# NIFTy-PPL/NIFTy

Measured on AMD Instinct MI355X. Metric: MGVI iters/sec on 1024^3 RGSpace CorrelatedField, 8 samples; achieved HBM GB/s, higher is better.
Workload: dtype f32

## Files before the change

__graft_entry__.py:

```python
import os
import subprocess
import sys

ROOT = os.path.dirname(os.path.abspath(__file__))
if ROOT not in sys.path:
    sys.path.insert(0, ROOT)


def build():
    csrc = os.path.join(ROOT, "nifty_amd", "csrc")
    subprocess.check_call(["make", "-C", csrc, "-j4", "ARCH=gfx950"])
    subprocess.check_call(["make", "-C", csrc, "fence", "ARCH=gfx950"])
    emu_dir = os.path.join(ROOT, "tests", "emu")
    subprocess.check_call(["g++", "-O2", "-std=c++17", "-shared", "-fPIC", "-o",
                           os.path.join(emu_dir, "libnk_emu.so"), os.path.join(emu_dir, "emu_fft.cpp"),
                           os.path.join(emu_dir, "emu_rng.cpp")])
    import oracle.nifty_oracle

    import nifty_amd
    from nifty_amd import _lib

    lib = _lib.load()
    assert lib.nk_version() >= 100


def smoke():
    import numpy as np
    import torch

    from nifty_amd import random
    from nifty_amd.engine import FusedKL, FusedModel, LatentVec, draw_samples
    from nifty_amd.minimization import AbsDeltaEnergyController
    from oracle import nifty_oracle as orc

    assert torch.cuda.is_available(), "smoke() needs a GPU"
    shape = (64, 64, 128)
    rng = np.random.default_rng(0)
    cf = orc.CFModel(shape, None, orc.CFParams(offset_mean=2.0))
    x = {k: 0.2 * v for k, v in cf.draw_latent(rng).items()}
    v = cf.draw_latent(rng)
    data = cf.forward(cf.draw_latent(rng)) + 0.1 * rng.normal(size=shape)
    lh = orc.Likelihood("gaussian", data, icov=100.0)
    lin = orc.Linearized(cf, lh, x)
    val, grad = lin.value_grad()
    mv = lin.metric(v)

    model = FusedModel(shape, offset_mean=2.0, likelihood="gaussian", data=data, icov=100.0, device="cuda:0")
    xl, vl = LatentVec.from_dict(model, x), LatentVec.from_dict(model, v)
    lp = model.linearize(xl)

    def rel(a, b):
        return max(float(np.max(np.abs(a[k] - b[k])) / max(np.max(np.abs(b[k])), 1e-30)) for k in ("xi", "spectrum"))

    assert abs(float(lp.value.item()) - val) < 1e-10 * abs(val)
    assert rel(lp.grad.to_dict(), grad) < 1e-9
    assert model.sandwich, "the sandwich pipeline should serve this grid"
    assert rel(model.metric(lp, vl).to_dict(), mv) < 1e-9
    random.push_sseq_from_seed(7)
    res, negs, n_total = draw_samples(model, xl, 1, True, lambda: AbsDeltaEnergyController(0.05, iteration_limit=5))
    random.pop_sseq()
    res_o, negs_o = orc.draw_samples(cf, lh, x, 1, True, np.random.SeedSequence(7),
                                     lambda: orc.AbsDeltaEnergyController(0.05, iteration_limit=5))
    assert rel(res[0].to_dict(), res_o[0]) < 1e-7
    kl = FusedKL(model, xl, res, negs)
    kl_o = orc.SampledKL(cf, lh, x, res_o, negs_o)
    assert abs(kl.value - kl_o.value) < 1e-8 * abs(kl_o.value)
    print("smoke OK: value", float(lp.value.item()), "KL", kl.value)


if __name__ == "__main__":
    build()
    print("build OK")
```

nifty_amd/csrc/nk_rng.h:

```cpp
#pragma once
#include <math.h>
#include <stdint.h>

#include "nk_core.h"
#include "nk_ziggurat_tables.h"

#define NK_RNG_CHUNK 64
#define NK_RNG_ERR_NOMERGE 1u
#define NK_RNG_ERR_SHORT 2u
#define NK_ZIG_R 3.6541528853610087963519472518
#define NK_ZIG_INV_R 0.27366123732975827203338247596

struct NkU128 {
  uint64_t hi, lo;
};
NK_HD uint64_t nk_mulhi64(uint64_t a, uint64_t b) {
#if defined(__HIP_DEVICE_COMPILE__)
  return __umul64hi(a, b);
#else
  return (uint64_t)(((unsigned __int128)a * b) >> 64);
#endif
}
NK_HD NkU128 nk_mul128(NkU128 a, NkU128 b) {
  NkU128 r;
  r.lo = a.lo * b.lo;
  r.hi = nk_mulhi64(a.lo, b.lo) + a.hi * b.lo + a.lo * b.hi;
  return r;
}
NK_HD NkU128 nk_add128(NkU128 a, NkU128 b) {
  NkU128 r;
  r.lo = a.lo + b.lo;
  r.hi = a.hi + b.hi + (r.lo < a.lo ? 1u : 0u);
  return r;
}

struct NkPcgJump {
  NkU128 m[64], p[64];
};
NK_HD void nk_pcg_jump_table(NkU128 inc, NkPcgJump& t) {
  NkU128 m{0x2360ED051FC65DA4ull, 0x4385DF649FCCF645ull}, p = inc;
  for (int i = 0; i < 64; ++i) {
    t.m[i] = m;
    t.p[i] = p;
    p = nk_mul128(nk_add128(m, NkU128{0, 1}), p);
    m = nk_mul128(m, m);
  }
}
NK_HD NkU128 nk_pcg_advance(NkU128 s, uint64_t delta, const NkPcgJump& t) {
  NkU128 am{0, 1}, ap{0, 0};
  for (int i = 0; delta; ++i, delta >>= 1)
    if (delta & 1) {
      am = nk_mul128(am, t.m[i]);
      ap = nk_add128(nk_mul128(ap, t.m[i]), t.p[i]);
    }
  return nk_add128(nk_mul128(am, s), ap);
}

struct NkRaw {
  NkU128 s, inc;
  int pos;
  NK_HD uint64_t next() {
    s = nk_add128(nk_mul128(s, NkU128{0x2360ED051FC65DA4ull, 0x4385DF649FCCF645ull}), inc);
    ++pos;
    const uint64_t x = s.hi ^ s.lo;
    const unsigned rot = (unsigned)(s.hi >> 58);
    return (x >> rot) | (x << ((64u - rot) & 63u));
  }
  NK_HD double next_double() { return (double)(next() >> 11) * (1.0 / 9007199254740992.0); }
};

struct NkZig {
  const uint64_t* ki;
  const double *wi, *fi;
};

#if defined(__clang__)
#define NK_NO_CONTRACT _Pragma("clang fp contract(off)")
#else
#define NK_NO_CONTRACT
#endif
#define NK_DMUL(a, b) ((a) * (b))
#define NK_DADD(a, b) ((a) + (b))

NK_HD double nk_zig_normal(NkRaw& g, const NkZig& z) {
  NK_NO_CONTRACT
  for (;;) {
    uint64_t r = g.next();
    const int idx = (int)(r & 0xff);
    r >>= 8;
    const int sign = (int)(r & 1);
    const uint64_t rabs = (r >> 1) & 0x000fffffffffffffull;
    double x = NK_DMUL((double)rabs, z.wi[idx]);
    if (sign) x = -x;
    if (rabs < z.ki[idx]) return x;
    if (idx == 0) {
      for (;;) {
        const double xx = NK_DMUL(-NK_ZIG_INV_R, log1p(-g.next_double()));
        const double yy = -log1p(-g.next_double());
        if (NK_DADD(yy, yy) > NK_DMUL(xx, xx)) return ((rabs >> 8) & 1) ? -NK_DADD(NK_ZIG_R, xx) : NK_DADD(NK_ZIG_R, xx);
      }
    } else {
      const double lhs = NK_DADD(NK_DMUL(z.fi[idx - 1] - z.fi[idx], g.next_double()), z.fi[idx]);
      if (lhs < exp(NK_DMUL(NK_DMUL(-0.5, x), x))) return x;
    }
  }
}

struct NkRngArgs {
  NkU128 state, inc;
  int64_t n;
  int64_t nchunks;
  double mean, std;
};

NK_HD NkRaw nk_rng_chunk_start(const NkRngArgs& a, const NkPcgJump& jt, int64_t k, int entry) {
  NkRaw g;
  g.inc = a.inc;
  g.s = nk_pcg_advance(a.state, (uint64_t)k * NK_RNG_CHUNK + (uint64_t)entry, jt);
  g.pos = entry;
  return g;
}

NK_HD void nk_rng_pass_a(const NkRngArgs& a, const NkPcgJump& jt, const NkZig& z, int64_t k, int& c0, int& ov, uint64_t& m) {
  NkRaw g = nk_rng_chunk_start(a, jt, k, 0);
  m = 0;
  c0 = 0;
  while (g.pos < NK_RNG_CHUNK) {
    m |= 1ull << g.pos;
    (void)nk_zig_normal(g, z);
    ++c0;
  }
  ov = g.pos - NK_RNG_CHUNK;
  if (ov > 255) ov = 255;
}

NK_HD int nk_rng_pass_a2(const NkRngArgs& a, const NkPcgJump& jt, const NkZig& z, int64_t k, int e, int c0, uint64_t m,
                         unsigned* err) {
  if (e == 0) return c0;
  if (e >= NK_RNG_CHUNK) {
    *err |= NK_RNG_ERR_NOMERGE;
    return 0;
  }
  NkRaw g = nk_rng_chunk_start(a, jt, k, e);
  int c = 0;
  while (g.pos < NK_RNG_CHUNK && !((m >> g.pos) & 1)) {
    (void)nk_zig_normal(g, z);
    ++c;
  }
  if (g.pos >= NK_RNG_CHUNK) {
    *err |= NK_RNG_ERR_NOMERGE;
    return 0;
  }
  int before = 0;
  for (int b = 0; b < g.pos; ++b) before += (int)((m >> b) & 1);
  return c + c0 - before;
}

template <typename T>
NK_HD void nk_rng_pass_b(const NkRngArgs& a, const NkPcgJump& jt, const NkZig& z, int64_t k, int entry, int64_t off, T* out,
                         uint64_t* consumed) {
  NK_NO_CONTRACT
  if (off >= a.n || entry >= NK_RNG_CHUNK) return;
  NkRaw g = nk_rng_chunk_start(a, jt, k, entry);
  while (g.pos < NK_RNG_CHUNK && off < a.n) {
    const double x = nk_zig_normal(g, z);
    out[off] = (T)NK_DADD(a.mean, NK_DMUL(a.std, x));
    if (off == a.n - 1) *consumed = (uint64_t)k * NK_RNG_CHUNK + (uint64_t)g.pos;
    ++off;
  }
}

static inline int64_t nk_rng_chunks_for(int64_t n, int attempt) {
  const double need = (double)n * (1.0225 + 0.005 * (double)(1 << attempt)) / NK_RNG_CHUNK;
  return (int64_t)need + 32 * (int64_t)(1 + attempt);
}

#define NK_RNG_FIX 32
template <typename T, int MODE>
NK_HD void nk_rng_fixed_body(NkU128 state, NkU128 inc, const NkPcgJump& jt, int64_t n, double low, double scale, int64_t k,
                             T* out) {
  NK_NO_CONTRACT
  const int64_t per = MODE == 0 ? NK_RNG_FIX : 2 * NK_RNG_FIX;
  const int64_t e0 = k * per;
  if (e0 >= n) return;
  NkRaw g;
  g.s = nk_pcg_advance(state, (uint64_t)k * NK_RNG_FIX, jt);
  g.inc = inc;
  g.pos = 0;
  for (int i = 0; i < NK_RNG_FIX; ++i) {
    const uint64_t raw = g.next();
    if (MODE == 0) {
      const int64_t e = e0 + i;
      if (e >= n) return;
      const double u = (double)(raw >> 11) * (1.0 / 9007199254740992.0);
      out[e] = (T)NK_DADD(low, NK_DMUL(scale, u));
    } else {
      for (int h = 0; h < 2; ++h) {
        const int64_t e = e0 + 2 * i + h;
        if (e >= n) return;
        const uint32_t half = h ? (uint32_t)(raw >> 32) : (uint32_t)raw;
        if (MODE == 1) {
          out[e] = (half >> 31) ? (T)1 : (T)-1;
        } else {
          const uint32_t code = half >> 30;
          out[2 * e] = code == 0 ? (T)1 : code == 2 ? (T)-1 : (T)0;
          out[2 * e + 1] = code == 1 ? (T)1 : code == 3 ? (T)-1 : (T)0;
        }
      }
    }
  }
}

struct NkIntArgs {
  NkU128 state, inc;
  int64_t n;
  uint64_t rng;
  int64_t low;
  int wide;
  uint64_t threshold;
};
NK_HD bool nk_int_accept(const NkIntArgs& a, uint64_t word, int64_t& value) {
  if (!a.wide) {
    const uint32_t excl = (uint32_t)a.rng + 1u;
    if (excl == 0u) {
      value = a.low + (int64_t)word;
      return true;
    }
    const uint64_t m = word * (uint64_t)excl;
    value = a.low + (int64_t)(m >> 32);
    return (uint32_t)m >= (uint32_t)a.threshold;
  }
  const uint64_t excl = a.rng + 1ull;
  if (excl == 0ull) {
    value = (int64_t)((uint64_t)a.low + word);
    return true;
  }
  const uint64_t lo = word * excl, hi = nk_mulhi64(word, excl);
  value = (int64_t)((uint64_t)a.low + hi);
  return lo >= a.threshold;
}
template <typename F>
NK_HD void nk_int_thread_words(const NkIntArgs& a, const NkPcgJump& jt, int64_t k, F f) {
  NkRaw g;
  g.s = nk_pcg_advance(a.state, (uint64_t)k * NK_RNG_FIX, jt);
  g.inc = a.inc;
  g.pos = 0;
  const int per = a.wide ? NK_RNG_FIX : 2 * NK_RNG_FIX;
  uint64_t raw = 0;
  for (int i = 0; i < per; ++i) {
    uint64_t word;
    if (a.wide) {
      word = g.next();
    } else {
      if ((i & 1) == 0) raw = g.next();
      word = (i & 1) ? (raw >> 32) : (raw & 0xffffffffull);
    }
    int64_t v;
    const bool ok = nk_int_accept(a, word, v);
    if (!f(k * per + i, ok, v)) return;
  }
}
NK_HD int nk_int_count(const NkIntArgs& a, const NkPcgJump& jt, int64_t k) {
  int c = 0;
  nk_int_thread_words(a, jt, k, [&](int64_t, bool ok, int64_t) {
    c += ok ? 1 : 0;
    return true;
  });
  return c;
}
NK_HD void nk_int_write(const NkIntArgs& a, const NkPcgJump& jt, int64_t k, int64_t off, int64_t* out, uint64_t* words_used) {
  nk_int_thread_words(a, jt, k, [&](int64_t word_index, bool ok, int64_t v) {
    if (!ok) return true;
    if (off >= a.n) return false;
    out[off] = v;
    if (off == a.n - 1) *words_used = (uint64_t)word_index + 1;
    ++off;
    return true;
  });
}
```

nifty_amd/csrc/nk_rng.hip:

```cpp
#include <hip/hip_runtime.h>

#include "nk_rng.h"
#include "nk_util.h"

namespace {

constexpr int RNG_THREADS = 256;

__device__ const uint64_t NK_ZIG_KI_DEV[256] = NK_ZIG_KI_INIT;
__device__ const uint64_t NK_ZIG_WI_DEV[256] = NK_ZIG_WI_BITS_INIT;
__device__ const uint64_t NK_ZIG_FI_DEV[256] = NK_ZIG_FI_BITS_INIT;

struct RngLds {
  NkPcgJump jt;
  uint64_t ki[256];
  double wi[256], fi[256];
};

__global__ void k_rng_table(NkU128 inc, NkPcgJump* out) {
  nk_pcg_jump_table(inc, *out);
}

__device__ __forceinline__ NkZig rng_load_lds(RngLds& l, const NkPcgJump* jt) {
  const uint64_t* src = (const uint64_t*)jt;
  uint64_t* dst = (uint64_t*)&l.jt;
  for (int i = threadIdx.x; i < (int)(sizeof(NkPcgJump) / 8); i += blockDim.x) dst[i] = src[i];
  for (int i = threadIdx.x; i < 256; i += blockDim.x) {
    l.ki[i] = NK_ZIG_KI_DEV[i];
    l.wi[i] = __longlong_as_double((long long)NK_ZIG_WI_DEV[i]);
    l.fi[i] = __longlong_as_double((long long)NK_ZIG_FI_DEV[i]);
  }
  __syncthreads();
  return NkZig{l.ki, l.wi, l.fi};
}

__global__ void __launch_bounds__(RNG_THREADS) k_rng_count(NkRngArgs a, const NkPcgJump* jt, uint8_t* over, uint8_t* cnt,
                                                           uint32_t* bsum, uint64_t* status) {
  __shared__ RngLds l;
  __shared__ int s_over[RNG_THREADS];
  __shared__ int s_sum[RNG_THREADS / 64];
  const NkZig z = rng_load_lds(l, jt);
  const int64_t k = (int64_t)blockIdx.x * RNG_THREADS + threadIdx.x;
  int c0 = 0, ov = 0;
  uint64_t m = 0;
  if (k < a.nchunks) nk_rng_pass_a(a, l.jt, z, k, c0, ov, m);
  s_over[threadIdx.x] = ov;
  __syncthreads();
  int c = 0;
  if (k < a.nchunks) {
    int e = 0;
    if (threadIdx.x > 0) {
      e = s_over[threadIdx.x - 1];
    } else if (k > 0) {
      int pc;
      uint64_t pm;
      nk_rng_pass_a(a, l.jt, z, k - 1, pc, e, pm);
    }
    unsigned err = 0;
    c = nk_rng_pass_a2(a, l.jt, z, k, e, c0, m, &err);
    if (err) atomicOr((unsigned long long*)&status[1], (unsigned long long)err);
    over[k] = (uint8_t)ov;
    cnt[k] = (uint8_t)c;
  }
  for (int d = 32; d > 0; d >>= 1) c += __shfl_down(c, d);
  if ((threadIdx.x & 63) == 0) s_sum[threadIdx.x >> 6] = c;
  __syncthreads();
  if (threadIdx.x == 0) {
    int t = 0;
    for (int w = 0; w < RNG_THREADS / 64; ++w) t += s_sum[w];
    bsum[blockIdx.x] = (uint32_t)t;
  }
}

__global__ void __launch_bounds__(1024) k_rng_scan(const uint32_t* bsum, int64_t nblk, int64_t n, int64_t* boff, uint64_t* status) {
  __shared__ int64_t part[1024];
  const int64_t seg = (nblk + 1023) / 1024;
  const int64_t lo = (int64_t)threadIdx.x * seg, hi = lo + seg < nblk ? lo + seg : nblk;
  int64_t s = 0;
  for (int64_t i = lo; i < hi; ++i) s += bsum[i];
  part[threadIdx.x] = s;
  __syncthreads();
  for (int d = 1; d < 1024; d <<= 1) {
    const int64_t v = threadIdx.x >= d ? part[threadIdx.x - d] : 0;
    __syncthreads();
    part[threadIdx.x] += v;
    __syncthreads();
  }
  int64_t run = part[threadIdx.x] - s;
  for (int64_t i = lo; i < hi; ++i) {
    boff[i] = run;
    run += bsum[i];
  }
  if (threadIdx.x == 1023 && part[1023] < n) atomicOr((unsigned long long*)&status[1], (unsigned long long)NK_RNG_ERR_SHORT);
}

template <typename T>
__global__ void __launch_bounds__(RNG_THREADS) k_rng_write(NkRngArgs a, const NkPcgJump* jt, const uint8_t* over, const uint8_t* cnt,
                                                           const int64_t* boff, T* out, uint64_t* status) {
  __shared__ RngLds l;
  __shared__ int s_scan[RNG_THREADS];
  const NkZig z = rng_load_lds(l, jt);
  const int64_t k = (int64_t)blockIdx.x * RNG_THREADS + threadIdx.x;
  const int c = k < a.nchunks ? cnt[k] : 0;
  s_scan[threadIdx.x] = c;
  __syncthreads();
  for (int d = 1; d < RNG_THREADS; d <<= 1) {
    const int v = threadIdx.x >= d ? s_scan[threadIdx.x - d] : 0;
    __syncthreads();
    s_scan[threadIdx.x] += v;
    __syncthreads();
  }
  if (k >= a.nchunks) return;
  const int64_t off = boff[blockIdx.x] + s_scan[threadIdx.x] - c;
  const int entry = k > 0 ? over[k - 1] : 0;
  nk_rng_pass_b<T>(a, l.jt, z, k, entry, off, out, &status[0]);
}

__global__ void __launch_bounds__(RNG_THREADS) k_int_count(NkIntArgs a, const NkPcgJump* jt, int64_t nthreads, uint8_t* cnt, uint32_t* bsum) {
  __shared__ NkPcgJump l_jt;
  __shared__ int s_sum[RNG_THREADS / 64];
  for (int i = threadIdx.x; i < (int)(sizeof(NkPcgJump) / sizeof(uint64_t)); i += blockDim.x)
    reinterpret_cast<uint64_t*>(&l_jt)[i] = reinterpret_cast<const uint64_t*>(jt)[i];
  __syncthreads();
  const int64_t k = (int64_t)blockIdx.x * RNG_THREADS + threadIdx.x;
  int c = 0;
  if (k < nthreads) {
    c = nk_int_count(a, l_jt, k);
    cnt[k] = (uint8_t)c;
  }
  for (int d = 32; d > 0; d >>= 1) c += __shfl_down(c, d);
  if ((threadIdx.x & 63) == 0) s_sum[threadIdx.x >> 6] = c;
  __syncthreads();
  if (threadIdx.x == 0) {
    int t = 0;
    for (int w = 0; w < RNG_THREADS / 64; ++w) t += s_sum[w];
    bsum[blockIdx.x] = (uint32_t)t;
  }
}
__global__ void __launch_bounds__(RNG_THREADS) k_int_write(NkIntArgs a, const NkPcgJump* jt, int64_t nthreads, const uint8_t* cnt,
                                                           const int64_t* boff, int64_t* out, uint64_t* status) {
  __shared__ NkPcgJump l_jt;
  __shared__ int s_scan[RNG_THREADS];
  for (int i = threadIdx.x; i < (int)(sizeof(NkPcgJump) / sizeof(uint64_t)); i += blockDim.x)
    reinterpret_cast<uint64_t*>(&l_jt)[i] = reinterpret_cast<const uint64_t*>(jt)[i];
  const int64_t k = (int64_t)blockIdx.x * RNG_THREADS + threadIdx.x;
  const int c = k < nthreads ? cnt[k] : 0;
  s_scan[threadIdx.x] = c;
  __syncthreads();
  for (int d = 1; d < RNG_THREADS; d <<= 1) {
    const int v = threadIdx.x >= d ? s_scan[threadIdx.x - d] : 0;
    __syncthreads();
    s_scan[threadIdx.x] += v;
    __syncthreads();
  }
  if (k >= nthreads) return;
  const int64_t off = boff[blockIdx.x] + s_scan[threadIdx.x] - c;
  if (off < a.n) nk_int_write(a, l_jt, k, off, out, &status[0]);
}

struct RngLayout {
  int64_t nchunks, nblk;
  int64_t o_over, o_cnt, o_bsum, o_boff, o_table, total;
};
RngLayout rng_layout(int64_t n, int attempt) {
  RngLayout L;
  L.nchunks = nk_rng_chunks_for(n, attempt);
  L.nblk = (L.nchunks + RNG_THREADS - 1) / RNG_THREADS;
  auto up = [](int64_t v) { return (v + 255) / 256 * 256; };
  L.o_over = 0;
  L.o_cnt = up(L.o_over + L.nchunks);
  L.o_bsum = up(L.o_cnt + L.nchunks);
  L.o_boff = up(L.o_bsum + 4 * L.nblk);
  L.o_table = up(L.o_boff + 8 * L.nblk);
  L.total = up(L.o_table + (int64_t)sizeof(NkPcgJump));
  return L;
}

template <typename T, int MODE>
__global__ void __launch_bounds__(256) k_rng_fixed(NkU128 state, NkU128 inc, const NkPcgJump* jt, int64_t n, double low,
                                                   double scale, T* out) {
  __shared__ NkPcgJump l_jt;
  for (int i = threadIdx.x; i < (int)(sizeof(NkPcgJump) / sizeof(uint64_t)); i += blockDim.x)
    reinterpret_cast<uint64_t*>(&l_jt)[i] = reinterpret_cast<const uint64_t*>(jt)[i];
  __syncthreads();
  nk_rng_fixed_body<T, MODE>(state, inc, l_jt, n, low, scale, (int64_t)blockIdx.x * blockDim.x + threadIdx.x, out);
}

template <int MODE>
int rng_fixed_launch(const uint64_t* state, const uint64_t* inc, int64_t n, double low, double scale, void* out, int dtype,
                     void* scratch, hipStream_t stream, const char* what) {
  if (!state || !inc || n < 0 || (n > 0 && (!out || !scratch)) || (dtype != NK_F32 && dtype != NK_F64))
    return nk_set_error(NK_ERR_INVALID, "nk_pcg64 fixed-rate draw: bad argument");
  if (!(inc[1] & 1)) return nk_set_error(NK_ERR_INVALID, "nk_pcg64 fixed-rate draw: the increment of a PCG64 stream is odd");
  if (n == 0) return NK_OK;
  const NkU128 s{state[0], state[1]}, c{inc[0], inc[1]};
  NkPcgJump* jt = (NkPcgJump*)scratch;
  hipLaunchKernelGGL(k_rng_table, dim3(1), dim3(1), 0, stream, c, jt);
  const int64_t per = MODE == 0 ? NK_RNG_FIX : 2 * NK_RNG_FIX;
  const int64_t threads = (n + per - 1) / per;
  const unsigned blocks = (unsigned)((threads + 255) / 256);
  if (dtype == NK_F32)
    hipLaunchKernelGGL((k_rng_fixed<float, MODE>), dim3(blocks), dim3(256), 0, stream, s, c, jt, n, low, scale, (float*)out);
  else
    hipLaunchKernelGGL((k_rng_fixed<double, MODE>), dim3(blocks), dim3(256), 0, stream, s, c, jt, n, low, scale, (double*)out);
  return nk_check_launch(what);
}

}

extern "C" int64_t nk_pcg64_fixed_scratch_bytes(void) { return (int64_t)sizeof(NkPcgJump); }

extern "C" int nk_pcg64_uniform(const uint64_t* state, const uint64_t* inc, int64_t n, double low, double high, void* out,
                                int dtype, void* scratch, void* stream) {
  return rng_fixed_launch<0>(state, inc, n, low, high - low, out, dtype, scratch, (hipStream_t)stream, "nk_pcg64_uniform");
}

extern "C" int nk_pcg64_pm1(const uint64_t* state, const uint64_t* inc, int64_t n, void* out, int dtype, int complex_units,
                            void* scratch, void* stream) {
  if (complex_units)
    return rng_fixed_launch<2>(state, inc, n, 0.0, 0.0, out, dtype, scratch, (hipStream_t)stream, "nk_pcg64_pm1");
  return rng_fixed_launch<1>(state, inc, n, 0.0, 0.0, out, dtype, scratch, (hipStream_t)stream, "nk_pcg64_pm1");
}

extern "C" int64_t nk_pcg64_integers_scratch_bytes(int64_t nthreads) {
  if (nthreads < 0) return 0;
  auto up = [](int64_t v) { return (v + 255) / 256 * 256; };
  const int64_t nblk = (nthreads + RNG_THREADS - 1) / RNG_THREADS;
  return up(nthreads) + up(4 * nblk) + up(8 * nblk) + up((int64_t)sizeof(NkPcgJump));
}

extern "C" int nk_pcg64_integers(const uint64_t* state, const uint64_t* inc, int64_t n, int64_t low, uint64_t rng, int64_t nthreads,
                                 int64_t* out, void* scratch, uint64_t* status, void* stream_) {
  hipStream_t stream = (hipStream_t)stream_;
  if (!state || !inc || n < 0 || nthreads < 0 || !status || (n > 0 && (!out || !scratch || nthreads < 1)) || rng == 0)
    return nk_set_error(NK_ERR_INVALID, "nk_pcg64_integers: bad argument (rng = high - low > 0)");
  if (!(inc[1] & 1)) return nk_set_error(NK_ERR_INVALID, "nk_pcg64_integers: the increment of a PCG64 stream is odd");
  hipError_t e = hipMemsetAsync(status, 0, 2 * sizeof(uint64_t), stream);
  if (e != hipSuccess) return nk_set_hip_error(e, "nk_pcg64_integers: hipMemsetAsync");
  if (n == 0) return NK_OK;
  NkIntArgs a;
  a.state = NkU128{state[0], state[1]};
  a.inc = NkU128{inc[0], inc[1]};
  a.n = n;
  a.rng = rng;
  a.low = low;
  a.wide = rng > 0xFFFFFFFFull ? 1 : 0;
  if (a.wide) a.threshold = rng == ~0ull ? 0 : (~0ull - rng) % (rng + 1ull);
  else a.threshold = rng == 0xFFFFFFFFull ? 0 : (0xFFFFFFFFull - rng) % (rng + 1ull);
  auto up = [](int64_t v) { return (v + 255) / 256 * 256; };
  const int64_t nblk = (nthreads + RNG_THREADS - 1) / RNG_THREADS;
  unsigned char* sc = (unsigned char*)scratch;
  uint8_t* cnt = sc;
  uint32_t* bsum = (uint32_t*)(sc + up(nthreads));
  int64_t* boff = (int64_t*)(sc + up(nthreads) + up(4 * nblk));
  NkPcgJump* jt = (NkPcgJump*)(sc + up(nthreads) + up(4 * nblk) + up(8 * nblk));
  hipLaunchKernelGGL(k_rng_table, dim3(1), dim3(1), 0, stream, a.inc, jt);
  hipLaunchKernelGGL(k_int_count, dim3((unsigned)nblk), dim3(RNG_THREADS), 0, stream, a, jt, nthreads, cnt, bsum);
  hipLaunchKernelGGL(k_rng_scan, dim3(1), dim3(1024), 0, stream, bsum, nblk, n, boff, status);
  hipLaunchKernelGGL(k_int_write, dim3((unsigned)nblk), dim3(RNG_THREADS), 0, stream, a, jt, nthreads, cnt, boff, out, status);
  return nk_check_launch("nk_pcg64_integers");
}

extern "C" int64_t nk_pcg64_normal_scratch_bytes(int64_t n, int attempt) {
  if (n < 0 || attempt < 0 || attempt > 8) return 0;
  return rng_layout(n, attempt).total;
}

extern "C" int nk_pcg64_normal(const uint64_t* state, const uint64_t* inc, int64_t n, double mean, double std, void* out,
                               int dtype, void* scratch, int64_t scratch_bytes, int attempt, uint64_t* status,
                               void* stream_) {
  hipStream_t stream = (hipStream_t)stream_;
  if (!state || !inc || n < 0 || !status || (n > 0 && (!out || !scratch)) || (dtype != NK_F32 && dtype != NK_F64) ||
      attempt < 0 || attempt > 8)
    return nk_set_error(NK_ERR_INVALID, "nk_pcg64_normal: bad argument");
  if (!(inc[1] & 1)) return nk_set_error(NK_ERR_INVALID, "nk_pcg64_normal: the increment of a PCG64 stream is odd");
  hipError_t e = hipMemsetAsync(status, 0, 2 * sizeof(uint64_t), stream);
  if (e != hipSuccess) return nk_set_hip_error(e, "nk_pcg64_normal: hipMemsetAsync");
  if (n == 0) return NK_OK;
  const RngLayout L = rng_layout(n, attempt);
  if (scratch_bytes < L.total) return nk_set_error(NK_ERR_INVALID, "nk_pcg64_normal: scratch smaller than nk_pcg64_normal_scratch_bytes");
  unsigned char* sc = (unsigned char*)scratch;
  NkRngArgs a;
  a.state = NkU128{state[0], state[1]};
  a.inc = NkU128{inc[0], inc[1]};
  a.n = n;
  a.nchunks = L.nchunks;
  a.mean = mean;
  a.std = std;
  NkPcgJump* jt = (NkPcgJump*)(sc + L.o_table);
  uint8_t* over = sc + L.o_over;
  uint8_t* cnt = sc + L.o_cnt;
  uint32_t* bsum = (uint32_t*)(sc + L.o_bsum);
  int64_t* boff = (int64_t*)(sc + L.o_boff);
  hipLaunchKernelGGL(k_rng_table, dim3(1), dim3(1), 0, stream, a.inc, jt);
  hipLaunchKernelGGL(k_rng_count, dim3((unsigned)L.nblk), dim3(RNG_THREADS), 0, stream, a, jt, over, cnt, bsum, status);
  hipLaunchKernelGGL(k_rng_scan, dim3(1), dim3(1024), 0, stream, bsum, L.nblk, n, boff, status);
  if (dtype == NK_F32)
    hipLaunchKernelGGL(k_rng_write<float>, dim3((unsigned)L.nblk), dim3(RNG_THREADS), 0, stream, a, jt, over, cnt, boff, (float*)out, status);
  else
    hipLaunchKernelGGL(k_rng_write<double>, dim3((unsigned)L.nblk), dim3(RNG_THREADS), 0, stream, a, jt, over, cnt, boff, (double*)out, status);
  return nk_check_launch("nk_pcg64_normal");
}
```

Baseline: 0.2225.

## Add wave-parallel PCG64 ziggurat normal sampler with ballot-based chunk chaining

Adds a new normal-sampling path where each of the 64 lanes of a wave evaluates one PCG64 output position of a 64-step chunk. Slow ziggurat attempts are resolved per lane, and the per-chunk accept masks are chained with ballots and shuffles. The old path had one thread walk a whole chunk serially, which caused heavy divergence and a long 128-bit multiply chain per thread; the new path replaces that with wide, mostly uniform work. It adds a mask buffer in scratch and segment-boundary consistency checks. The old chunk path remains available through an environment variable.

```diff
diff --git a/__graft_entry__.py b/__graft_entry__.py
--- a/__graft_entry__.py
+++ b/__graft_entry__.py
@@ -15,6 +15,8 @@
     subprocess.check_call(["g++", "-O2", "-std=c++17", "-shared", "-fPIC", "-o",
                            os.path.join(emu_dir, "libnk_emu.so"), os.path.join(emu_dir, "emu_fft.cpp"),
                            os.path.join(emu_dir, "emu_rng.cpp")])
+    subprocess.check_call(["g++", "-O2", "-std=c++17", "-shared", "-fPIC", "-o",
+                           os.path.join(emu_dir, "libnk_emu_rngw.so"), os.path.join(emu_dir, "emu_rng_wave.cpp")])
     import oracle.nifty_oracle
 
     import nifty_amd
diff --git a/nifty_amd/csrc/nk_rng.h b/nifty_amd/csrc/nk_rng.h
--- a/nifty_amd/csrc/nk_rng.h
+++ b/nifty_amd/csrc/nk_rng.h
@@ -168,6 +168,110 @@
     if (off == a.n - 1) *consumed = (uint64_t)k * NK_RNG_CHUNK + (uint64_t)g.pos;
     ++off;
   }
+}
+
+
+NK_HD NkU128 nk_pcg_jump(NkU128 s, uint64_t delta, const NkPcgJump& t) {
+  for (int i = 0; delta; ++i, delta >>= 1)
+    if (delta & 1) s = nk_add128(nk_mul128(s, t.m[i]), t.p[i]);
+  return s;
+}
+NK_HD uint64_t nk_pcg_output(NkU128 s) {
+  const uint64_t x = s.hi ^ s.lo;
+  const unsigned rot = (unsigned)(s.hi >> 58);
+  return (x >> rot) | (x << ((64u - rot) & 63u));
+}
+NK_HD NkU128 nk_rngw_group_base(const NkRngArgs& a, const NkPcgJump& jt, int64_t group) {
+  return nk_pcg_jump(a.state, (uint64_t)group * NK_RNG_CHUNK, jt);
+}
+NK_HD NkU128 nk_rngw_lane_start(NkU128 base, const NkPcgJump& jt, int lane) { return nk_pcg_jump(base, (uint64_t)lane + 1u, jt); }
+NK_HD NkU128 nk_rngw_lane_next(NkU128 s, const NkPcgJump& jt) { return nk_add128(nk_mul128(s, jt.m[6]), jt.p[6]); }
+
+NK_HD double nk_rngw_tail(NkU128 s, NkU128 inc, int& len) {
+  NK_NO_CONTRACT
+  NkRaw g;
+  g.s = s;
+  g.inc = inc;
+  g.pos = 1;
+  for (;;) {
+    const double xx = NK_DMUL(-NK_ZIG_INV_R, log1p(-g.next_double()));
+    const double yy = -log1p(-g.next_double());
+    if (NK_DADD(yy, yy) > NK_DMUL(xx, xx)) {
+      len = g.pos;
+      return xx;
+    }
+  }
+}
+
+struct NkAttempt {
+  int slow, yield, tail, len;
+};
+NK_HD bool nk_rngw_is_slow(uint64_t r, const NkZig& z) { return !(((r >> 9) & 0x000fffffffffffffull) < z.ki[r & 0xff]); }
+NK_HD NkAttempt nk_rngw_slow_attempt(NkU128 s, NkU128 inc, const NkZig& z) {
+  NK_NO_CONTRACT
+  const uint64_t r = nk_pcg_output(s);
+  const int idx = (int)(r & 0xff);
+  NkAttempt t{1, 1, 0, 2};
+  if (idx == 0) {
+    t.tail = 1;
+    (void)nk_rngw_tail(s, inc, t.len);
+  } else {
+    const uint64_t rabs = (r >> 9) & 0x000fffffffffffffull;
+    const double x = NK_DMUL((double)rabs, z.wi[idx]);
+    NkRaw g;
+    g.s = s;
+    g.inc = inc;
+    g.pos = 0;
+    const double lhs = NK_DADD(NK_DMUL(z.fi[idx - 1] - z.fi[idx], g.next_double()), z.fi[idx]);
+    t.yield = lhs < exp(NK_DMUL(NK_DMUL(-0.5, x), x)) ? 1 : 0;
+  }
+  return t;
+}
+
+template <typename TailLen>
+NK_HD void nk_rngw_chain(uint64_t slow, uint64_t yield, uint64_t tail, int entry, TailLen tail_len, uint64_t& out, int& over) {
+  out = 0;
+  int pos = entry;
+  while (pos < NK_RNG_CHUNK) {
+    const uint64_t rest = slow >> pos;
+    if (!rest) {
+      out |= ~0ull << pos;
+      pos = NK_RNG_CHUNK;
+      break;
+    }
+    const int q = pos + __builtin_ctzll(rest);
+    out |= (~0ull << pos) & ((1ull << q) - 1ull);
+    out |= yield & (1ull << q);
+    const int len = ((tail >> q) & 1ull) ? tail_len(q) : 2;
+    pos = q + (len > 1 ? len : 1);
+  }
+  over = pos - NK_RNG_CHUNK;
+}
+NK_HD unsigned nk_rngw_boundary_err(int over_true, int over_zero) { return over_true == over_zero ? 0u : NK_RNG_ERR_NOMERGE; }
+
+NK_HD double nk_rngw_value(NkU128 s, NkU128 inc, const NkZig& z) {
+  NK_NO_CONTRACT
+  uint64_t r = nk_pcg_output(s);
+  const int idx = (int)(r & 0xff);
+  r >>= 8;
+  const int sign = (int)(r & 1);
+  const uint64_t rabs = (r >> 1) & 0x000fffffffffffffull;
+  if (idx == 0 && !(rabs < z.ki[0])) {
+    int len;
+    const double xx = nk_rngw_tail(s, inc, len);
+    return ((rabs >> 8) & 1) ? -NK_DADD(NK_ZIG_R, xx) : NK_DADD(NK_ZIG_R, xx);
+  }
+  const double x = NK_DMUL((double)rabs, z.wi[idx]);
+  return sign ? -x : x;
+}
+NK_HD int nk_rngw_length(NkU128 s, NkU128 inc, const NkZig& z) {
+  if (!nk_rngw_is_slow(nk_pcg_output(s), z)) return 1;
+  return nk_rngw_slow_attempt(s, inc, z).len;
+}
+template <typename T>
+NK_HD T nk_rngw_scaled(const NkRngArgs& a, double x) {
+  NK_NO_CONTRACT
+  return (T)NK_DADD(a.mean, NK_DMUL(a.std, x));
 }
 
 static inline int64_t nk_rng_chunks_for(int64_t n, int attempt) {
diff --git a/nifty_amd/csrc/nk_rng.hip b/nifty_amd/csrc/nk_rng.hip
--- a/nifty_amd/csrc/nk_rng.hip
+++ b/nifty_amd/csrc/nk_rng.hip
@@ -1,4 +1,6 @@
 #include <hip/hip_runtime.h>
+#include <stdlib.h>
+#include <string.h>
 
 #include "nk_rng.h"
 #include "nk_util.h"
@@ -114,6 +116,96 @@
   const int64_t off = boff[blockIdx.x] + s_scan[threadIdx.x] - c;
   const int entry = k > 0 ? over[k - 1] : 0;
   nk_rng_pass_b<T>(a, l.jt, z, k, entry, off, out, &status[0]);
+}
+
+constexpr int RNGW_G = 64;
+constexpr int RNGW_WAVES = RNG_THREADS / 64;
+
+template <int G>
+__global__ void __launch_bounds__(RNG_THREADS) k_rngw_decide(NkRngArgs a, const NkPcgJump* jt, uint64_t* masks, uint32_t* segcnt,
+                                                             uint32_t* bsum, uint64_t* status) {
+  __shared__ RngLds l;
+  __shared__ int s_sum[RNGW_WAVES];
+  const NkZig z = rng_load_lds(l, jt);
+  const int lane = threadIdx.x & 63, wave = threadIdx.x >> 6;
+  const int64_t seg = (int64_t)blockIdx.x * RNGW_WAVES + wave;
+  const int64_t g0 = seg * G, g1 = g0 + G < a.nchunks ? g0 + G : a.nchunks;
+  int count = 0;
+  if (g0 < g1) {
+    const int64_t gfirst = g0 > 0 ? g0 - 1 : 0;
+    NkU128 s = nk_rngw_lane_start(nk_rngw_group_base(a, l.jt, gfirst), l.jt, lane);
+    int entry = 0;
+    for (int64_t g = gfirst; g < g1; ++g) {
+      const bool slow = nk_rngw_is_slow(nk_pcg_output(s), z);
+      const uint64_t m_slow = __ballot(slow);
+      uint64_t m_yield = 0, m_tail = 0;
+      int len = 2;
+      if (m_slow) {
+        NkAttempt t{0, 0, 0, 2};
+        if (slow) t = nk_rngw_slow_attempt(s, a.inc, z);
+        m_yield = __ballot(t.slow && t.yield);
+        m_tail = __ballot(t.slow && t.tail);
+        len = t.len;
+      }
+      auto tail_len = [&](int q) { return __shfl(len, q); };
+      uint64_t out;
+      int over;
+      nk_rngw_chain(m_slow, m_yield, m_tail, entry, tail_len, out, over);
+      if (g >= g0) {
+        if (lane == 0) masks[g] = out;
+        count += __popcll(out);
+        if (g == g0 + G - 1 && g + 1 < a.nchunks && entry != 0) {
+          uint64_t out0;
+          int over0;
+          nk_rngw_chain(m_slow, m_yield, m_tail, 0, tail_len, out0, over0);
+          const unsigned err = nk_rngw_boundary_err(over, over0);
+          if (err && lane == 0) atomicOr((unsigned long long*)&status[1], (unsigned long long)err);
+        }
+      }
+      entry = over;
+      s = nk_rngw_lane_next(s, l.jt);
+    }
+  }
+  if (lane == 0) {
+    segcnt[seg] = (uint32_t)count;
+    s_sum[wave] = count;
+  }
+  __syncthreads();
+  if (threadIdx.x == 0) {
+    int t = 0;
+    for (int w = 0; w < RNGW_WAVES; ++w) t += s_sum[w];
+    bsum[blockIdx.x] = (uint32_t)t;
+  }
+}
+
+template <typename T, int G>
+__global__ void __launch_bounds__(RNG_THREADS) k_rngw_write(NkRngArgs a, const NkPcgJump* jt, const uint64_t* masks,
+                                                            const uint32_t* segcnt, const int64_t* boff, T* out, uint64_t* status) {
+  __shared__ RngLds l;
+  const NkZig z = rng_load_lds(l, jt);
+  const int lane = threadIdx.x & 63, wave = threadIdx.x >> 6;
+  const int64_t seg = (int64_t)blockIdx.x * RNGW_WAVES + wave;
+  const int64_t g0 = seg * G, g1 = g0 + G < a.nchunks ? g0 + G : a.nchunks;
+  if (g0 >= g1) return;
+  int64_t off = boff[blockIdx.x];
+  for (int w = 0; w < wave; ++w) off += segcnt[seg - wave + w];
+  if (off >= a.n) return;
+  NkU128 s = nk_rngw_lane_start(nk_rngw_group_base(a, l.jt, g0), l.jt, lane);
+  uint64_t mine = 0;
+  for (int64_t g = g0; g < g1 && off < a.n; ++g) {
+    const int w = (int)(g - g0) & 63;
+    if (w == 0) mine = g + lane < g1 ? masks[g + lane] : 0;
+    const uint64_t m = ((uint64_t)(uint32_t)__shfl((int)(mine >> 32), w) << 32) | (uint32_t)__shfl((int)mine, w);
+    if ((m >> lane) & 1ull) {
+      const int64_t dest = off + __popcll(m & ((1ull << lane) - 1ull));
+      if (dest < a.n) {
+        out[dest] = nk_rngw_scaled<T>(a, nk_rngw_value(s, a.inc, z));
+        if (dest == a.n - 1) status[0] = (uint64_t)g * NK_RNG_CHUNK + (uint64_t)lane + (uint64_t)nk_rngw_length(s, a.inc, z);
+      }
+    }
+    off += __popcll(m);
+    s = nk_rngw_lane_next(s, l.jt);
+  }
 }
 
 __global__ void __launch_bounds__(RNG_THREADS) k_int_count(NkIntArgs a, const NkPcgJump* jt, int64_t nthreads, uint8_t* cnt, uint32_t* bsum) {
@@ -174,6 +266,33 @@
   L.o_table = up(L.o_boff + 8 * L.nblk);
   L.total = up(L.o_table + (int64_t)sizeof(NkPcgJump));
   return L;
+}
+
+struct RngWaveLayout {
+  int64_t ngroups, nblk;
+  int64_t o_mask, o_segcnt, o_bsum, o_boff, o_table, total;
+};
+RngWaveLayout rngw_layout(int64_t n, int attempt) {
+  RngWaveLayout L;
+  L.ngroups = nk_rng_chunks_for(n, attempt);
+  const int64_t nseg = (L.ngroups + RNGW_G - 1) / RNGW_G;
+  L.nblk = (nseg + RNGW_WAVES - 1) / RNGW_WAVES;
+  auto up = [](int64_t v) { return (v + 255) / 256 * 256; };
+  L.o_mask = 0;
+  L.o_segcnt = up(L.o_mask + 8 * L.ngroups);
+  L.o_bsum = up(L.o_segcnt + 4 * RNGW_WAVES * L.nblk);
+  L.o_boff = up(L.o_bsum + 4 * L.nblk);
+  L.o_table = up(L.o_boff + 8 * L.nblk);
+  L.total = up(L.o_table + (int64_t)sizeof(NkPcgJump));
+  return L;
+}
+
+constexpr int64_t RNGW_MIN_N = 0;
+bool rng_walk_is_chunk(int64_t n) {
+  const char* v = getenv("NK_RNG_WALK");
+  if (v && strcmp(v, "chunk") == 0) return true;
+  if (v && strcmp(v, "wave") == 0) return false;
+  return n < RNGW_MIN_N;
 }
 
 template <typename T, int MODE>
@@ -263,7 +382,8 @@
 
 extern "C" int64_t nk_pcg64_normal_scratch_bytes(int64_t n, int attempt) {
   if (n < 0 || attempt < 0 || attempt > 8) return 0;
-  return rng_layout(n, attempt).total;
+  const int64_t chunk = rng_layout(n, attempt).total, wave = rngw_layout(n, attempt).total;
+  return chunk > wave ? chunk : wave;
 }
 
 extern "C" int nk_pcg64_normal(const uint64_t* state, const uint64_t* inc, int64_t n, double mean, double std, void* out,
@@ -277,16 +397,34 @@
   hipError_t e = hipMemsetAsync(status, 0, 2 * sizeof(uint64_t), stream);
   if (e != hipSuccess) return nk_set_hip_error(e, "nk_pcg64_normal: hipMemsetAsync");
   if (n == 0) return NK_OK;
-  const RngLayout L = rng_layout(n, attempt);
-  if (scratch_bytes < L.total) return nk_set_error(NK_ERR_INVALID, "nk_pcg64_normal: scratch smaller than nk_pcg64_normal_scratch_bytes");
+  if (scratch_bytes < nk_pcg64_normal_scratch_bytes(n, attempt))
+    return nk_set_error(NK_ERR_INVALID, "nk_pcg64_normal: scratch smaller than nk_pcg64_normal_scratch_bytes");
   unsigned char* sc = (unsigned char*)scratch;
   NkRngArgs a;
   a.state = NkU128{state[0], state[1]};
   a.inc = NkU128{inc[0], inc[1]};
   a.n = n;
-  a.nchunks = L.nchunks;
   a.mean = mean;
   a.std = std;
+  if (!rng_walk_is_chunk(n)) {
+    const RngWaveLayout W = rngw_layout(n, attempt);
+    a.nchunks = W.ngroups;
+    NkPcgJump* jt = (NkPcgJump*)(sc + W.o_table);
+    uint64_t* masks = (uint64_t*)(sc + W.o_mask);
+    uint32_t* segcnt = (uint32_t*)(sc + W.o_segcnt);
+    uint32_t* bsum = (uint32_t*)(sc + W.o_bsum);
+    int64_t* boff = (int64_t*)(sc + W.o_boff);
+    hipLaunchKernelGGL(k_rng_table, dim3(1), dim3(1), 0, stream, a.inc, jt);
+    hipLaunchKernelGGL(k_rngw_decide<RNGW_G>, dim3((unsigned)W.nblk), dim3(RNG_THREADS), 0, stream, a, jt, masks, segcnt, bsum, status);
+    hipLaunchKernelGGL(k_rng_scan, dim3(1), dim3(1024), 0, stream, bsum, W.nblk, n, boff, status);
+    if (dtype == NK_F32)
+      hipLaunchKernelGGL((k_rngw_write<float, RNGW_G>), dim3((unsigned)W.nblk), dim3(RNG_THREADS), 0, stream, a, jt, masks, segcnt, boff, (float*)out, status);
+    else
+      hipLaunchKernelGGL((k_rngw_write<double, RNGW_G>), dim3((unsigned)W.nblk), dim3(RNG_THREADS), 0, stream, a, jt, masks, segcnt, boff, (double*)out, status);
+    return nk_check_launch("nk_pcg64_normal");
+  }
+  const RngLayout L = rng_layout(n, attempt);
+  a.nchunks = L.nchunks;
   NkPcgJump* jt = (NkPcgJump*)(sc + L.o_table);
   uint8_t* over = sc + L.o_over;
   uint8_t* cnt = sc + L.o_cnt;
```

New measurement: 0.2239, median of 6. No clear change (+0.6%).
